# Shinokawa/Fast-SCNN-pytorch

Hardware: AMD Instinct MI355X
Metric: images/sec fwd+bwd @1024x2048 bs=8 per GPU; 1/2/4/8-GPU scaling (higher is better)
Workload: dtype bf16; 1 GPU; cfg3 train step: fwd + CE(ignore -1) + bwd + fused SGD (fused low-res upsample+CE head); model=FastSCNN (19 classes), global_batch=8, per_gpu_batch=8, parallelism=dp1

## Files before the change

fast-scnn-pytorch_amd/csrc/gemm_stream.hip:

```cpp
#include "bn_finish.hpp"

namespace fscnn {

constexpr int GS_MW = 32;
constexpr int GS_KMAX = 576;

template <typename T>
struct GsMma;
template <>
struct GsMma<float> {
  static __device__ __forceinline__ void run(const uint4& w, const uint4& x, f32x4& acc) {
    acc = __builtin_amdgcn_mfma_f32_16x16x4f32(__uint_as_float(w.x), __uint_as_float(x.x), acc, 0, 0, 0);
    acc = __builtin_amdgcn_mfma_f32_16x16x4f32(__uint_as_float(w.y), __uint_as_float(x.y), acc, 0, 0, 0);
    acc = __builtin_amdgcn_mfma_f32_16x16x4f32(__uint_as_float(w.z), __uint_as_float(x.z), acc, 0, 0, 0);
    acc = __builtin_amdgcn_mfma_f32_16x16x4f32(__uint_as_float(w.w), __uint_as_float(x.w), acc, 0, 0, 0);
  }
};
template <>
struct GsMma<bf16> {
  static __device__ __forceinline__ void run(const uint4& w, const uint4& x, f32x4& acc) {
    i16x8 wv, xv;
    __builtin_memcpy(&wv, &w, 16);
    __builtin_memcpy(&xv, &x, 16);
    acc = __builtin_amdgcn_mfma_f32_16x16x32_bf16(wv, xv, acc, 0, 0, 0);
  }
};
template <>
struct GsMma<f16> {
  static __device__ __forceinline__ void run(const uint4& w, const uint4& x, f32x4& acc) {
    h16x8 wv, xv;
    __builtin_memcpy(&wv, &w, 16);
    __builtin_memcpy(&xv, &x, 16);
    acc = __builtin_amdgcn_mfma_f32_16x16x32_f16(wv, xv, acc, 0, 0, 0);
  }
};

template <typename T>
__device__ __forceinline__ uint4 gs_tail(uint4 v, int valid) {
  constexpr int V = VecW<T>::V;
  uint32_t w[4] = {v.x, v.y, v.z, v.w};
#pragma unroll
  for (int j = 0; j < 4; ++j) {
    if (V == 4) {
      w[j] = j < valid ? w[j] : 0u;
    } else {
      const uint32_t lo = (2 * j < valid) ? 0x0000FFFFu : 0u;
      const uint32_t hi = (2 * j + 1 < valid) ? 0xFFFF0000u : 0u;
      w[j] &= lo | hi;
    }
  }
  return make_uint4(w[0], w[1], w[2], w[3]);
}

__device__ __forceinline__ float gs_rowsum(float v) {
  v += __shfl_xor(v, 1);
  v += __shfl_xor(v, 2);
  v += __shfl_xor(v, 4);
  v += __shfl_xor(v, 8);
  return v;
}

constexpr int GS_TEAM = 16;
constexpr int GS_CTR_TEAMS = 64;

template <bool FWD>
__device__ inline void gs_fold(const GemmArgs& a, int n0, int BN, int first, int count, int stride,
                               double (&sum)[3]) {
  __shared__ double s_f[3][256];
  const int tid = threadIdx.x;
  const int S = 256 / BN;
  const int col = tid % BN, sl = tid / BN;
  const int n = n0 + col;
  const int N = a.N;
  const float* base = FWD ? a.part : a.bpart;
  constexpr int R = FWD ? 3 : 2;
  constexpr int U = FWD ? 8 : 4;
  double t0 = 0.0, t1 = 0.0, t2 = 0.0;
  if (sl < S && n < N) {
    for (int i0 = sl; i0 < count; i0 += U * S) {
      float v[U][R];
#pragma unroll
      for (int u = 0; u < U; ++u) {
        const int i = i0 + u * S;
        const float* rec = base + (size_t)(first + (i < count ? i : i0) * stride) * R * N;
#pragma unroll
        for (int j = 0; j < R; ++j) v[u][j] = ld_wt(rec + (size_t)j * N + n);
      }
#pragma unroll
      for (int u = 0; u < U; ++u) {
        if (i0 + u * S >= count) break;
        if constexpr (FWD) {
          const double cn = v[u][2], m = v[u][0];
          t0 += cn;
          t1 += cn * m;
          t2 += (double)v[u][1] + cn * m * m;
        } else {
          t1 += v[u][0];
          t2 += v[u][1];
        }
      }
    }
  }
  s_f[0][tid] = t0;
  s_f[1][tid] = t1;
  s_f[2][tid] = t2;
  __syncthreads();
  sum[0] = sum[1] = sum[2] = 0.0;
  if (sl == 0) {
    for (int j = 0; j < S; ++j) {
      sum[0] += s_f[0][j * BN + col];
      sum[1] += s_f[1][j * BN + col];
      sum[2] += s_f[2][j * BN + col];
    }
  }
  __syncthreads();
}

template <bool FWD>
__device__ inline void gs_finish(const GemmArgs& a, int g, int bi, int n0, int BN, int bpg) {
  unsigned* ctr = a.tail.counters;
  const int team = bi / GS_TEAM, nteam = cdiv(bpg, GS_TEAM);
  const int tsize = min(GS_TEAM, bpg - team * GS_TEAM);
  const int tid = threadIdx.x, col = tid % BN, n = n0 + col;
  const bool owner = tid < BN && n < a.N;
  if (!arrive_last(ctr + GS_CTR_TEAMS + g * nteam + team, (unsigned)tsize)) return;
  BnFwdIn fin;
  BnBwdIn bin;
  if (owner) {
    if constexpr (FWD) fin = bn_fwd_load(a.tail.fwd, n);
    else bin = bn_bwd_load(a.tail.tab, n);
  }
  double s[3];
  gs_fold<FWD>(a, n0, BN, team * GS_TEAM, tsize, 1, s);
  if (owner) {
    const int N = a.N;
    if constexpr (FWD) {
      float* rec = a.part + (size_t)team * GS_TEAM * 3 * N;
      const double mean = s[0] > 0.0 ? s[1] / s[0] : 0.0;
      st_wt(rec + n, (float)mean);
      st_wt(rec + N + n, s[0] > 0.0 ? (float)fmax(s[2] - s[0] * mean * mean, 0.0) : 0.f);
      st_wt(rec + 2 * N + n, (float)s[0]);
    } else {
      float* rec = a.bpart + (size_t)team * GS_TEAM * 2 * N;
      st_wt(rec + n, (float)s[1]);
      st_wt(rec + N + n, (float)s[2]);
    }
  }
  reset_counter(ctr + GS_CTR_TEAMS + g * nteam + team);
  if (!arrive_last(ctr + g, (unsigned)nteam)) return;
  gs_fold<FWD>(a, n0, BN, 0, nteam, GS_TEAM, s);
  if (owner) {
    if constexpr (FWD) bn_fwd_finish(a.tail.fwd, n, s[0], s[1], s[2], fin);
    else bn_bwd_finish(n, a.N, s[1], s[2], a.tail.count, a.tail.dgamma, a.tail.dbeta,
                       a.tail.coef, a.tail.tab, bin);
  }
  reset_counter(ctr + g);
}

template <typename T, int NT, int KS, bool TAIL, bool AT, bool ST, bool BS>
__global__ __launch_bounds__(256, 2) void gemm_stream_kernel(GemmArgs a, int bpg) {
  constexpr int V = VecW<T>::V;
  constexpr int KV = 4 * KS;
  constexpr int KP = KV * V;
  constexpr int WST = KV + 1;
  constexpr int BN = 16 * NT;
  constexpr bool SUMS = ST || BS;
  extern __shared__ __attribute__((aligned(16))) uint4 s_w[];
  float* s_sc = reinterpret_cast<float*>(s_w + BN * WST);
  float* s_at = s_sc + 2 * BN;
  float* s_bc = s_at + (AT ? 2 * KP : 0);
  float* s_shf = s_bc + (BS ? 4 * BN : 0);

  const int tid = threadIdx.x, lane = tid & 63, wave = tid >> 6;
  const int li = lane & 15, lq = lane >> 4;
  const int g = blockIdx.x / bpg;
  const int bi = blockIdx.x - g * bpg;
  const int n0 = g * BN;
  const T* A = (const T*)a.A;
  const T* B = (const T*)a.B;
  stamp(a.stamps, 0);

  const int nchunks = cdiv(a.M, GS_MW);
  const int wstride = bpg * 4;
  int c = bi * 4 + wave;

  constexpr int NH =
      KS <= 4 ? 1 : (KS <= 8 ? 2 : (KS == 12 ? (BS ? 4 : 2) : (KS == 16 ? 4 : 6)));
  constexpr int KH = KS / NH;
  static_assert(KH * NH == KS && (NH == 1 || NH % 2 == 0), "k-steps split in an even part count");
  uint4 xa[2][KH], xn[2][KH];
  auto loadx = [&](int chunk, int h, uint4 (&r)[2][KH]) {
    const bool cok = chunk < nchunks;
#pragma unroll
    for (int mt = 0; mt < 2; ++mt) {
      const int m = chunk * GS_MW + mt * 16 + li;
      const bool mok = cok && m < a.M;
#pragma unroll
      for (int j = 0; j < KH; ++j) {
        const int k = (4 * (h * KH + j) + lq) * V;
        const bool ok = mok && k < a.K;
        r[mt][j] = *reinterpret_cast<const uint4*>(A + (ok ? (size_t)m * a.lda + k : 0));
      }
    }
  };

  if (c < nchunks) loadx(c, 0, xa);
  float t_sc = 1.f, t_sh = 0.f, t_bc[4] = {0.f, 0.f, 0.f, 1.f};
  if (tid < BN) {
    const int n = n0 + tid < a.N ? n0 + tid : 0;
    if (a.scale) t_sc = a.scale[n];
    if (a.shift) t_sh = a.shift[n];
    if constexpr (BS) {
      t_bc[0] = a.bmean[n];
      t_bc[1] = a.binvstd[n];
      if (a.bmode == 2) {
        t_bc[2] = a.bscale[n];
        t_bc[3] = a.bshift[n];
      }
    }
  }
  constexpr int ATI = AT ? (KP + 255) / 256 : 1;
  float t_at[ATI][2];
  if constexpr (AT) {
#pragma unroll
    for (int u = 0; u < ATI; ++u) {
      const int k = tid + u * 256;
      const bool ok = k < a.K;
      t_at[u][0] = ok ? a.a_scale[k] : 0.f;
      t_at[u][1] = ok ? a.a_shift[k] : 0.f;
    }
  }
  constexpr int WI = (BN * KV + 255) / 256;
  constexpr int WB = WI < 8 ? WI : 8;
#pragma unroll
  for (int u0 = 0; u0 < WI; u0 += WB) {
    uint4 t[WB];
#pragma unroll
    for (int u = 0; u < WB; ++u) {
      const int i = tid + (u0 + u) * 256;
      const int r = i / KV, v = i - r * KV;
      const int n = n0 + r, k = v * V;
      const bool ok = u0 + u < WI && i < BN * KV && n < a.N && k < a.K;
      t[u] = gs_tail<T>(*reinterpret_cast<const uint4*>(B + (ok ? (size_t)n * a.ldb + k : 0)),
                        ok ? a.K - k : 0);
    }
#pragma unroll
    for (int u = 0; u < WB; ++u) {
      const int i = tid + (u0 + u) * 256;
      const int r = i / KV, v = i - r * KV;
      if (u0 + u < WI && i < BN * KV) s_w[r * WST + v] = t[u];
    }
  }
  if (tid < BN) {
    s_sc[tid] = t_sc;
    s_sc[BN + tid] = t_sh;
    if constexpr (BS) {
#pragma unroll
      for (int j = 0; j < 4; ++j) s_bc[j * BN + tid] = t_bc[j];
    }
  }
  if constexpr (AT) {
#pragma unroll
    for (int u = 0; u < ATI; ++u) {
      const int k = tid + u * 256;
      if (k < KP) {
        s_at[k] = t_at[u][0];
        s_at[KP + k] = t_at[u][1];
      }
    }
  }
  __syncthreads();
  stamp(a.stamps, 1);

  float s1[SUMS ? NT : 1][4], s2[SUMS ? NT : 1][4];
  float cnt = 0.f;
  if constexpr (SUMS) {
#pragma unroll
    for (int nt = 0; nt < NT; ++nt)
#pragma unroll
      for (int r = 0; r < 4; ++r) { s1[nt][r] = 0.f; s2[nt][r] = 0.f; }
  }
  float* wshf = s_shf + wave * BN;
  if constexpr (ST) {
    for (int i = lane; i < BN; i += 64) wshf[i] = 0.f;
  }
  bool first = true;

  auto prep = [&](int chunk, int h, uint4 (&r)[2][KH]) {
#pragma unroll
    for (int mt = 0; mt < 2; ++mt) {
      const int m = chunk * GS_MW + mt * 16 + li;
      const bool mok = m < a.M;
#pragma unroll
      for (int j = 0; j < KH; ++j) {
        const int k = (4 * (h * KH + j) + lq) * V;
        uint4 v = r[mt][j];
        if constexpr (AT) v = bnrelu_vec<T>(v, s_at + k, s_at + KP + k);
        r[mt][j] = gs_tail<T>(v, mok ? a.K - k : 0);
      }
    }
  };

  T* Cp = (T*)a.C;
  const T* Rp = (const T*)a.R;
  constexpr bool DROP_OK = BS && KS == 1;
  const bool drop = DROP_OK && a.drop_hw != 0;
  const uint64_t dseed = drop ? (a.drop_seed_ptr ? *a.drop_seed_ptr : a.drop_seed) + a.drop_seed_add : 0;
  const float dscale = 1.f / (1.f - a.drop_p);
  for (; c < nchunks; c += wstride) {
    f32x4 acc[2][NT];
#pragma unroll
    for (int mt = 0; mt < 2; ++mt)
#pragma unroll
      for (int nt = 0; nt < NT; ++nt) acc[mt][nt] = f32x4{0.f, 0.f, 0.f, 0.f};
    int wb = li * WST + lq;
    asm volatile("" : "+v"(wb));
    const int wz = wb - li * WST - lq;
    const float* ssc = s_sc + wz;
    const float* sbc = s_bc + wz;
    auto mma = [&](int h, uint4 (&r)[2][KH]) {
#pragma unroll
      for (int j = 0; j < KH; ++j) {
#pragma unroll
        for (int nt = 0; nt < NT; ++nt) {
          const uint4 w = s_w[wb + nt * 16 * WST + 4 * (h * KH + j)];
#pragma unroll
          for (int mt = 0; mt < 2; ++mt) GsMma<T>::run(w, r[mt][j], acc[mt][nt]);
        }
      }
    };
    if constexpr (NH == 1) {
      loadx(c + wstride, 0, xn);
      prep(c, 0, xa);
      mma(0, xa);
    } else {
#pragma unroll
      for (int h = 0; h < NH; h += 2) {
        loadx(c, h + 1, xn);
        prep(c, h, xa);
        mma(h, xa);
        if (h + 2 < NH) loadx(c, h + 2, xa);
        else loadx(c + wstride, 0, xa);
        prep(c, h + 1, xn);
        mma(h + 1, xn);
      }
    }
    if constexpr (!TAIL) {
      if constexpr (ST) {
        if (first) {
          if (li == 0) {
#pragma unroll
            for (int nt = 0; nt < NT; ++nt) {
              const int nl = nt * 16 + 4 * lq;
#pragma unroll
              for (int r = 0; r < 4; ++r) wshf[nl + r] = acc[0][nt][r] * ssc[nl + r] + ssc[BN + nl + r];
            }
          }
          __builtin_amdgcn_wave_barrier();
          first = false;
        }
      }
#pragma unroll
      for (int mt = 0; mt < 2; ++mt) {
        const int m = c * GS_MW + mt * 16 + li;
        const bool mok = m < a.M;
        const size_t mr = mok ? (size_t)m : 0;
        float rv[NT][4];
        if (Rp) {
#pragma unroll
          for (int nt = 0; nt < NT; ++nt) ld4v(Rp + mr * a.ldr + n0 + nt * 16 + 4 * lq, rv[nt]);
        }
        float zv[BS ? NT : 1][4];
        if constexpr (BS) {
#pragma unroll
          for (int nt = 0; nt < NT; ++nt)
            ld4v((const T*)a.bz + mr * a.ldbz + n0 + nt * 16 + 4 * lq, zv[nt]);
        }
        if constexpr (SUMS) cnt += mok ? 1.f : 0.f;
#pragma unroll
        for (int nt = 0; nt < NT; ++nt) {
          const int nl = nt * 16 + 4 * lq;
          const float4 sc = *reinterpret_cast<const float4*>(ssc + nl);
          const float4 sh = *reinterpret_cast<const float4*>(ssc + BN + nl);
          const float scv[4] = {sc.x, sc.y, sc.z, sc.w}, shv[4] = {sh.x, sh.y, sh.z, sh.w};
          float shf[4] = {0.f, 0.f, 0.f, 0.f};
          if constexpr (ST) {
            const float4 t = *reinterpret_cast<const float4*>(wshf + wz + nl);
            shf[0] = t.x; shf[1] = t.y; shf[2] = t.z; shf[3] = t.w;
          }
          float o[4];
#pragma unroll
          for (int r = 0; r < 4; ++r) {
            float v = acc[mt][nt][r] * scv[r] + shv[r];
            if constexpr (ST) {
              const float d = mok ? round_as<T>(v) - shf[r] : 0.f;
              s1[nt][r] += d;
              s2[nt][r] += d * d;
            }
            if (Rp) v += rv[nt][r];
            o[r] = a.relu ? fmaxf(v, 0.f) : v;
          }
          if (DROP_OK && drop) {
            const unsigned HW = (unsigned)a.drop_hw;
            const unsigned pn = (unsigned)mr / HW, hw = (unsigned)mr - pn * HW;
#pragma unroll
            for (int r = 0; r < 4; ++r) {
              const uint64_t nchw = ((uint64_t)pn * a.N + (unsigned)(n0 + nl + r)) * HW + hw;
              o[r] = dropout_keep(dseed, nchw, a.drop_thr) ? round_as<T>(o[r]) * dscale : 0.f;
            }
          }
          if (mok) st4v(Cp + mr * a.ldc + n0 + nl, o);
          if constexpr (BS) {
            const float4 bm = *reinterpret_cast<const float4*>(sbc + nl);
            const float4 bv = *reinterpret_cast<const float4*>(sbc + BN + nl);
            const float4 bs = *reinterpret_cast<const float4*>(sbc + 2 * BN + nl);
            const float4 bh = *reinterpret_cast<const float4*>(sbc + 3 * BN + nl);
            const float bmv[4] = {bm.x, bm.y, bm.z, bm.w}, biv[4] = {bv.x, bv.y, bv.z, bv.w};
            const float bsv[4] = {bs.x, bs.y, bs.z, bs.w}, bhv[4] = {bh.x, bh.y, bh.z, bh.w};
#pragma unroll
            for (int r = 0; r < 4; ++r) {
              float gv = round_as<T>(o[r]);
              gv = (mok && fmaf(zv[nt][r], bsv[r], bhv[r]) > 0.f) ? gv : 0.f;
              s1[nt][r] += gv;
              s2[nt][r] += gv * (zv[nt][r] - bmv[r]) * biv[r];
            }
          }
        }
      }
    } else {
#pragma unroll
      for (int mt = 0; mt < 2; ++mt) {
        const int m = c * GS_MW + mt * 16 + li;
        if (m >= a.M) continue;
#pragma unroll
        for (int nt = 0; nt < NT; ++nt) {
          const int nl = nt * 16 + 4 * lq;
#pragma unroll
          for (int r = 0; r < 4; ++r) {
            const int n = n0 + nl + r;
            if (n >= a.N) continue;
            float v = acc[mt][nt][r] * ssc[nl + r] + ssc[BN + nl + r];
            if (Rp) v += ld1(Rp + (size_t)m * a.ldr + n);
            st1(Cp + (size_t)m * a.ldc + n, a.relu ? fmaxf(v, 0.f) : v);
          }
        }
      }
    }
    if constexpr (NH == 1) {
#pragma unroll
      for (int mt = 0; mt < 2; ++mt)
#pragma unroll
        for (int j = 0; j < KH; ++j) xa[mt][j] = xn[mt][j];
    }
  }

  stamp(a.stamps, 2);
  if constexpr (SUMS) {
    cnt = gs_rowsum(cnt);
    __syncthreads();
    float* red = reinterpret_cast<float*>(s_w);
#pragma unroll
    for (int nt = 0; nt < NT; ++nt)
#pragma unroll
      for (int r = 0; r < 4; ++r) {
        const float t1 = gs_rowsum(s1[nt][r]), t2 = gs_rowsum(s2[nt][r]);
        if (li == 0) {
          const int col = nt * 16 + 4 * lq + r;
          if constexpr (ST) {
            const float mean = cnt > 0.f ? wshf[col] + t1 / cnt : 0.f;
            const float m2 = cnt > 0.f ? fmaxf(t2 - t1 * (t1 / cnt), 0.f) : 0.f;
            red[(wave * 3 + 0) * BN + col] = cnt;
            red[(wave * 3 + 1) * BN + col] = mean;
            red[(wave * 3 + 2) * BN + col] = m2;
          } else {
            red[(wave * 3 + 0) * BN + col] = t1;
            red[(wave * 3 + 1) * BN + col] = t2;
          }
        }
      }
    __syncthreads();
    for (int col = tid; col < BN; col += 256) {
      const int n = n0 + col;
      if (n >= a.N) continue;
      if constexpr (ST) {
        float nn = 0.f, mean = 0.f, m2 = 0.f;
#pragma unroll
        for (int w = 0; w < 4; ++w) {
          const float nb = red[(w * 3 + 0) * BN + col];
          if (nb <= 0.f) continue;
          const float mb = red[(w * 3 + 1) * BN + col], qb = red[(w * 3 + 2) * BN + col];
          const float tot = nn + nb, d = mb - mean;
          mean += d * (nb / tot);
          m2 += qb + d * d * (nn * nb / tot);
          nn = tot;
        }
        float* rec = a.part + (size_t)bi * 3 * a.N;
        st_wt(rec + n, mean);
        st_wt(rec + a.N + n, m2);
        st_wt(rec + 2 * a.N + n, nn);
      } else {
        float t1 = 0.f, t2 = 0.f;
#pragma unroll
        for (int w = 0; w < 4; ++w) {
          t1 += red[(w * 3 + 0) * BN + col];
          t2 += red[(w * 3 + 1) * BN + col];
        }
        float* rec = a.bpart + (size_t)bi * 2 * a.N;
        st_wt(rec + n, t1);
        st_wt(rec + a.N + n, t2);
      }
    }
    stamp(a.stamps, 3);
    if (a.tail.counters) gs_finish<ST>(a, g, bi, n0, BN, bpg);
    stamp(a.stamps, 4);
  }
}

template <int NT, int KS, bool TAIL>
__global__ __launch_bounds__(256, 2) void gemm_stream_x3_kernel(GemmArgs a, int bpg) {
  constexpr int KV = 4 * KS;
  constexpr int WST = KV + 1;
  constexpr int BN = 16 * NT;
  extern __shared__ __attribute__((aligned(16))) uint4 s_w[];
  float* s_sc = reinterpret_cast<float*>(s_w + 3 * BN * WST);
  const int tid = threadIdx.x, lane = tid & 63, wave = tid >> 6;
  const int li = lane & 15, lq = lane >> 4;
  const int g = blockIdx.x / bpg;
  const int bi = blockIdx.x - g * bpg;
  const int n0 = g * BN;
  const float* A = (const float*)a.A;
  const float* B = (const float*)a.B;
  for (int i = tid; i < BN * KV; i += 256) {
    const int r = i / KV, v = i - r * KV;
    const int n = n0 + r, k = v * 8;
    const bool ok = n < a.N && k < a.K;
    const float* src = B + (ok ? (size_t)n * a.ldb + k : 0);
    const uint4 lo4 = gs_tail<float>(*reinterpret_cast<const uint4*>(src), ok ? a.K - k : 0);
    const uint4 hi4 = gs_tail<float>(*reinterpret_cast<const uint4*>(src + 4), ok ? a.K - k - 4 : 0);
    uint4 t[3];
    gs_split3(lo4, hi4, t);
#pragma unroll
    for (int j = 0; j < 3; ++j) s_w[(j * BN + r) * WST + v] = t[j];
  }
  for (int i = tid; i < BN; i += 256) {
    const int n = n0 + i < a.N ? n0 + i : 0;
    s_sc[i] = a.scale ? a.scale[n] : 1.f;
    s_sc[BN + i] = a.shift ? a.shift[n] : 0.f;
  }
  __syncthreads();

  const int nchunks = cdiv(a.M, GS_MW);
  const int wstride = bpg * 4;
  int c = bi * 4 + wave;
  uint4 xa[2][KS][2], xn[2][KS][2];
  auto loadx = [&](int chunk, uint4 (&r)[2][KS][2]) {
    const bool cok = chunk < nchunks;
#pragma unroll
    for (int mt = 0; mt < 2; ++mt) {
      const int m = chunk * GS_MW + mt * 16 + li;
      const bool mok = cok && m < a.M;
#pragma unroll
      for (int s = 0; s < KS; ++s)
#pragma unroll
        for (int h = 0; h < 2; ++h) {
          const int k = 32 * s + 8 * lq + 4 * h;
          const bool ok = mok && k < a.K;
          r[mt][s][h] = *reinterpret_cast<const uint4*>(A + (ok ? (size_t)m * a.lda + k : 0));
        }
    }
  };
  float* Cp = (float*)a.C;
  const float* Rp = (const float*)a.R;
  if (c < nchunks) loadx(c, xa);
  for (; c < nchunks; c += wstride) {
    loadx(c + wstride, xn);
    f32x4 acc[2][NT];
#pragma unroll
    for (int mt = 0; mt < 2; ++mt)
#pragma unroll
      for (int nt = 0; nt < NT; ++nt) acc[mt][nt] = f32x4{0.f, 0.f, 0.f, 0.f};
    int wb = li * WST + lq;
    asm volatile("" : "+v"(wb));
    const float* ssc = s_sc + (wb - li * WST - lq);
#pragma unroll
    for (int s = 0; s < KS; ++s) {
      uint4 xs[2][3];
#pragma unroll
      for (int mt = 0; mt < 2; ++mt) {
        const int m = c * GS_MW + mt * 16 + li;
        const bool mok = m < a.M;
        const int k = 32 * s + 8 * lq;
        gs_split3(gs_tail<float>(xa[mt][s][0], mok ? a.K - k : 0),
                  gs_tail<float>(xa[mt][s][1], mok ? a.K - k - 4 : 0), xs[mt]);
      }
#pragma unroll
      for (int nt = 0; nt < NT; ++nt) {
        uint4 w[3];
#pragma unroll
        for (int j = 0; j < 3; ++j) w[j] = s_w[(j * BN + nt * 16) * WST + wb + 4 * s];
#pragma unroll
        for (int mt = 0; mt < 2; ++mt) gs_mma_x3(w, xs[mt], acc[mt][nt]);
      }
    }
#pragma unroll
    for (int mt = 0; mt < 2; ++mt) {
      const int m = c * GS_MW + mt * 16 + li;
      const bool mok = m < a.M;
      const size_t mr = mok ? (size_t)m : 0;
      if constexpr (!TAIL) {
        float rv[NT][4];
        if (Rp) {
#pragma unroll
          for (int nt = 0; nt < NT; ++nt) ld4v(Rp + mr * a.ldr + n0 + nt * 16 + 4 * lq, rv[nt]);
        }
#pragma unroll
        for (int nt = 0; nt < NT; ++nt) {
          const int nl = nt * 16 + 4 * lq;
          float o[4];
#pragma unroll
          for (int r = 0; r < 4; ++r) {
            float v = acc[mt][nt][r] * ssc[nl + r] + ssc[BN + nl + r];
            if (Rp) v += rv[nt][r];
            o[r] = a.relu ? fmaxf(v, 0.f) : v;
          }
          if (mok) st4v(Cp + mr * a.ldc + n0 + nl, o);
        }
      } else {
        if (!mok) continue;
#pragma unroll
        for (int nt = 0; nt < NT; ++nt) {
          const int nl = nt * 16 + 4 * lq;
#pragma unroll
          for (int r = 0; r < 4; ++r) {
            const int n = n0 + nl + r;
            if (n >= a.N) continue;
            float v = acc[mt][nt][r] * ssc[nl + r] + ssc[BN + nl + r];
            if (Rp) v += ld1(Rp + (size_t)m * a.ldr + n);
            st1(Cp + (size_t)m * a.ldc + n, a.relu ? fmaxf(v, 0.f) : v);
          }
        }
      }
    }
#pragma unroll
    for (int mt = 0; mt < 2; ++mt)
#pragma unroll
      for (int s = 0; s < KS; ++s)
#pragma unroll
        for (int h = 0; h < 2; ++h) xa[mt][s][h] = xn[mt][s][h];
  }
}

static int gs_st_nt_cap() {
  static const int v = env_int("FSCNN_GS_ST_NT", 4);
  return v;
}

static int gs_pick_nt(const GemmArgs& a, int ks) {
  const int N = a.N;
  if (N <= 32) return 2;
  if (a.part && ks <= 8 && N > 64 && gs_st_nt_cap() > 0) {
    for (int nt = gs_st_nt_cap(); nt >= 2; --nt)
      if (N % (16 * nt) == 0) return nt;
  }
  if (ks > 8) return N % 64 == 0 ? 4 : (N % 48 == 0 ? 3 : 4);
  if (N <= 48) return 3;
  if (N <= 64 || a.bpart) return 4;
  if (a.part && ks > 2 && N % 64 == 0) return 4;
  if (N % 96 == 0) return 6;
  return a.part ? 4 : 8;
}

static bool gs_tail_needed(const GemmArgs& a, int nt) {
  return a.N % (16 * nt) != 0 || a.ldc % 4 != 0 || (a.R && a.ldr % 4 != 0);
}

static size_t gs_lds(const GemmArgs& a, int nt, int ks, int kc) {
  size_t b = (size_t)16 * nt * (4 * ks + 1) * 16 + (size_t)2 * 16 * nt * 4;
  if (a.a_scale) b += (size_t)2 * ks * kc * 4;
  if (a.bpart) b += (size_t)4 * 16 * nt * 4;
  if (a.part) b += (size_t)4 * 16 * nt * 4;
  return b;
}

static int gs_bpg(const GemmArgs& a, int dtype, int& nt, int& ks, size_t& lds);

bool gemm_stream_ok(const GemmArgs& a, int dtype) {
  const int KC = dtype == DT_F32 ? 16 : 32;
  const int ks = cdiv(a.K, KC);
  const bool sums = a.part || a.bpart;
  if (a.b_trans || (a.part && a.bpart)) return false;
  if (a.part && a.R) return false;
  if (a.a_scale && (!a.a_shift || !a.part || a.K > GS_KMAX)) return false;
  const bool deep = ks == 12 || ks == 16 || ks == 18;
  if (deep && dtype == DT_F32) return false;
  if (deep && a.M < 131072) return false;
  if (!(ks == 1 || ks == 2 || ks == 3 || ks == 4 || ks == 6 || ks == 8 || deep)) return false;
  const int nt = gs_pick_nt(a, ks);
  if (sums && ks > 4 && nt > 4) return false;
  if (sums && nt == 4 && ks > 12) return false;
  if (a.part && nt > 4 && ks > 2) return false;
  if (a.bpart && dtype == DT_F32 && nt == 4 && ks > 2) return false;
  if (gs_tail_needed(a, nt) && (nt != 2 || sums)) return false;
  if (a.bpart && (!a.bz || a.ldbz % 4 || (a.bmode != 0 && a.bmode != 2))) return false;
  if (a.drop_hw && (!a.bpart || ks != 1 || gs_tail_needed(a, nt) || a.M % a.drop_hw)) return false;
  if (gs_lds(a, nt, ks, KC) > (deep ? 80 * 1024 - 1024 : 72 * 1024)) return false;
  if (a.tail.counters) {
    int nt2, ks2;
    size_t lds2;
    const int bpg = gs_bpg(a, dtype, nt2, ks2, lds2);
    const int groups = cdiv(a.N, 16 * nt);
    if (groups > GS_CTR_TEAMS || GS_CTR_TEAMS + groups * cdiv(bpg, GS_TEAM) > BN_COUNTERS)
      return false;
  }
  return a.M >= 4096;
}

static int gs_fill_bpg(int slots, int groups) {
  const int b = slots / groups / 8 * 8;
  return b >= 8 ? b : (cdiv(slots, groups) + 7) / 8 * 8;
}

static int gs_bpg(const GemmArgs& a, int dtype, int& nt, int& ks, size_t& lds) {
  const int KC = dtype == DT_F32 ? 16 : 32;
  ks = cdiv(a.K, KC);
  nt = gs_pick_nt(a, ks);
  const int groups = cdiv(a.N, 16 * nt);
  lds = gs_lds(a, nt, ks, KC);
  const int nchunks = cdiv(a.M, GS_MW);
  constexpr int cap = 2;
  int per_cu = (int)((160 * 1024) / (lds + 1024));
  per_cu = per_cu < 1 ? 1 : (per_cu > cap ? cap : per_cu);
  int bpg = gs_fill_bpg(256 * per_cu, groups);
  const int need = cdiv(nchunks, 4);
  if (bpg > need) bpg = need;
  const int tmax = (BN_COUNTERS - GS_CTR_TEAMS) / groups * GS_TEAM;
  if (bpg > tmax) bpg = tmax;
  if (bpg < 1) bpg = 1;
  return bpg;
}

int gemm_stream_parts(const GemmArgs& a, int dtype) {
  int nt, ks;
  size_t lds;
  return gs_bpg(a, dtype, nt, ks, lds);
}

template <typename T, int NT, bool TAIL, bool AT, bool ST, bool BS>
static void gs_launch_ks(const GemmArgs& a, int ks, dim3 grid, size_t lds, int bpg,
                         hipStream_t st) {
  constexpr bool SUMS = ST || BS;
  constexpr bool WIDE = SUMS && NT > 4;
  constexpr bool DEEP = sizeof(T) == 2 && NT <= 4 && !TAIL;
  switch (ks) {
    case 1: prof_launch(gemm_stream_kernel<T, NT, 1, TAIL, AT, ST, BS>, grid, 256, lds, st, a, bpg); break;
    case 2: prof_launch(gemm_stream_kernel<T, NT, 2, TAIL, AT, ST, BS>, grid, 256, lds, st, a, bpg); break;
    case 3:
      if constexpr (!WIDE) prof_launch(gemm_stream_kernel<T, NT, 3, TAIL, AT, ST, BS>, grid, 256, lds, st, a, bpg);
      break;
    case 4:
      if constexpr (!WIDE) prof_launch(gemm_stream_kernel<T, NT, 4, TAIL, AT, ST, BS>, grid, 256, lds, st, a, bpg);
      break;
    case 6:
      if constexpr (!WIDE) prof_launch(gemm_stream_kernel<T, NT, 6, TAIL, AT, ST, BS>, grid, 256, lds, st, a, bpg);
      break;
    case 8:
      if constexpr (!WIDE) prof_launch(gemm_stream_kernel<T, NT, 8, TAIL, AT, ST, BS>, grid, 256, lds, st, a, bpg);
      break;
    default:
      if constexpr (DEEP) {
        if (ks == 12) prof_launch(gemm_stream_kernel<T, NT, 12, TAIL, AT, ST, BS>, grid, 256, lds, st, a, bpg);
        else if (ks == 16) prof_launch(gemm_stream_kernel<T, NT, 16, TAIL, AT, ST, BS>, grid, 256, lds, st, a, bpg);
        else prof_launch(gemm_stream_kernel<T, NT, 18, TAIL, AT, ST, BS>, grid, 256, lds, st, a, bpg);
      }
      break;
  }
}

template <typename T, bool AT, bool ST, bool BS>
static void gs_launch_nt(const GemmArgs& a, int nt, int ks, dim3 grid, size_t lds, int bpg,
                         hipStream_t st) {
  constexpr bool SUMS = ST || BS;
  switch (nt) {
    case 2:
      if (!SUMS && gs_tail_needed(a, nt)) gs_launch_ks<T, 2, true, AT, false, false>(a, ks, grid, lds, bpg, st);
      else gs_launch_ks<T, 2, false, AT, ST, BS>(a, ks, grid, lds, bpg, st);
      break;
    case 3: gs_launch_ks<T, 3, false, AT, ST, BS>(a, ks, grid, lds, bpg, st); break;
    case 4: gs_launch_ks<T, 4, false, AT, ST, BS>(a, ks, grid, lds, bpg, st); break;
    case 6:
      if constexpr (!BS) gs_launch_ks<T, 6, false, AT, ST, false>(a, ks, grid, lds, bpg, st);
      break;
    default:
      if constexpr (!SUMS) gs_launch_ks<T, 8, false, AT, false, false>(a, ks, grid, lds, bpg, st);
      break;
  }
}

template <typename T>
static void gs_launch(const GemmArgs& a, int dtype, hipStream_t st) {
  int nt, ks;
  size_t lds;
  const int bpg = gs_bpg(a, dtype, nt, ks, lds);
  const int groups = cdiv(a.N, 16 * nt);
  dim3 grid((unsigned)(groups * bpg));
  const bool at = a.a_scale != nullptr;
  if (a.bpart) gs_launch_nt<T, false, false, true>(a, nt, ks, grid, lds, bpg, st);
  else if (a.part && at) gs_launch_nt<T, true, true, false>(a, nt, ks, grid, lds, bpg, st);
  else if (a.part) gs_launch_nt<T, false, true, false>(a, nt, ks, grid, lds, bpg, st);
  else gs_launch_nt<T, false, false, false>(a, nt, ks, grid, lds, bpg, st);
}

static bool gs_x3_launch(const GemmArgs& a, hipStream_t st) {
  if (!f32_split_on() || a.part || a.bpart || a.a_scale || a.K > 128) return false;
  const int ks = cdiv(a.K, 32);
  auto lds_of = [&](int nt) { return (size_t)3 * 16 * nt * (4 * ks + 1) * 16 + (size_t)2 * 16 * nt * 4; };
  int nt = gs_pick_nt(a, ks);
  while (nt > 2 && lds_of(nt) > 72 * 1024) nt = nt == 8 ? 4 : (nt == 6 ? 3 : 2);
  if (lds_of(nt) > 72 * 1024) return false;
  const bool tail = gs_tail_needed(a, nt);
  if (tail && nt != 2) return false;
  const size_t lds = lds_of(nt);
  const int groups = cdiv(a.N, 16 * nt);
  int per_cu = (int)((160 * 1024) / (lds + 1024));
  per_cu = per_cu < 1 ? 1 : (per_cu > 2 ? 2 : per_cu);
  int bpg = gs_fill_bpg(256 * per_cu, groups);
  const int need = cdiv(cdiv(a.M, GS_MW), 4);
  if (bpg > need) bpg = need;
  if (bpg < 1) bpg = 1;
  const dim3 grid((unsigned)(groups * bpg));
#define X3(NT, KS, TL) prof_launch(gemm_stream_x3_kernel<NT, KS, TL>, grid, 256, lds, st, a, bpg)
#define X3K(NT, TL)                         \
  switch (ks) {                             \
    case 1: X3(NT, 1, TL); break;           \
    case 2: X3(NT, 2, TL); break;           \
    case 3: X3(NT, 3, TL); break;           \
    default: X3(NT, 4, TL); break;          \
  }
  switch (nt) {
    case 2: if (tail) { X3K(2, true) } else { X3K(2, false) } break;
    case 3: X3K(3, false) break;
    case 4: X3K(4, false) break;
    case 6: X3K(6, false) break;
    default: X3K(8, false) break;
  }
#undef X3K
#undef X3
  return true;
}

int gemm_stream(const GemmArgs& a, int dtype, hipStream_t st) {
  if (dtype == DT_F32) {
    if (!gs_x3_launch(a, st)) gs_launch<float>(a, dtype, st);
  } else if (dtype == DT_F16) {
    gs_launch<f16>(a, dtype, st);
  } else {
    gs_launch<bf16>(a, dtype, st);
  }
  return check_launch("gemm_stream");
}

}
```

Measured before the change: 1462 images/s.

## Add prefetching bf16 stream-GEMM variant for backward-stat kernels with 32-bit offsets

Adds a specialized gemm_stream_kernel_pf for bf16, non-tail, BS (backward stats) cases with KS<=12. It issues the epilogue operand loads (bz and residual rows) for the current chunk, and the next chunk's A loads, early so they overlap the MFMA work. Address arithmetic uses 32-bit offsets when the host check confirms the tensors fit under 4 GiB, and the epilogue uses vectorized row loads and stores. The added prefetch registers raise register pressure and may lower occupancy, and the code duplication adds maintenance cost.

```diff
diff --git a/fast-scnn-pytorch_amd/csrc/gemm_stream.hip b/fast-scnn-pytorch_amd/csrc/gemm_stream.hip
--- a/fast-scnn-pytorch_amd/csrc/gemm_stream.hip
+++ b/fast-scnn-pytorch_amd/csrc/gemm_stream.hip
@@ -2,6 +2,7 @@
 
 namespace fscnn {
 
+#define GS_INLINE __attribute__((always_inline))
 constexpr int GS_MW = 32;
 constexpr int GS_KMAX = 576;
 
@@ -50,6 +51,35 @@
     }
   }
   return make_uint4(w[0], w[1], w[2], w[3]);
+}
+
+template <typename P>
+__device__ __forceinline__ const P* gs_at(const P* base, uint32_t off) {
+  return reinterpret_cast<const P*>(reinterpret_cast<const char*>(base) +
+                                    (size_t)(off * (uint32_t)sizeof(P)));
+}
+template <typename P>
+__device__ __forceinline__ P* gs_at(P* base, uint32_t off) {
+  return reinterpret_cast<P*>(reinterpret_cast<char*>(base) + (size_t)(off * (uint32_t)sizeof(P)));
+}
+
+template <typename T> struct GsRow { using type = uint2; };
+template <> struct GsRow<float> { using type = uint4; };
+template <typename T>
+__device__ __forceinline__ typename GsRow<T>::type gs_row_load(const T* p) {
+  return *reinterpret_cast<const typename GsRow<T>::type*>(p);
+}
+__device__ __forceinline__ void gs_row_unpack(const float*, const uint4& t, float (&v)[4]) {
+  v[0] = __uint_as_float(t.x); v[1] = __uint_as_float(t.y);
+  v[2] = __uint_as_float(t.z); v[3] = __uint_as_float(t.w);
+}
+__device__ __forceinline__ void gs_row_unpack(const f16*, const uint2& t, float (&v)[4]) {
+  v[0] = h2f((uint16_t)(t.x & 0xFFFFu)); v[1] = h2f((uint16_t)(t.x >> 16));
+  v[2] = h2f((uint16_t)(t.y & 0xFFFFu)); v[3] = h2f((uint16_t)(t.y >> 16));
+}
+__device__ __forceinline__ void gs_row_unpack(const bf16*, const uint2& t, float (&v)[4]) {
+  v[0] = __uint_as_float(t.x << 16); v[1] = __uint_as_float(t.x & 0xFFFF0000u);
+  v[2] = __uint_as_float(t.y << 16); v[3] = __uint_as_float(t.y & 0xFFFF0000u);
 }
 
 __device__ __forceinline__ float gs_rowsum(float v) {
@@ -453,6 +483,380 @@
         for (int j = 0; j < KH; ++j) xa[mt][j] = xn[mt][j];
     }
   }
+
+  stamp(a.stamps, 2);
+  if constexpr (SUMS) {
+    cnt = gs_rowsum(cnt);
+    __syncthreads();
+    float* red = reinterpret_cast<float*>(s_w);
+#pragma unroll
+    for (int nt = 0; nt < NT; ++nt)
+#pragma unroll
+      for (int r = 0; r < 4; ++r) {
+        const float t1 = gs_rowsum(s1[nt][r]), t2 = gs_rowsum(s2[nt][r]);
+        if (li == 0) {
+          const int col = nt * 16 + 4 * lq + r;
+          if constexpr (ST) {
+            const float mean = cnt > 0.f ? wshf[col] + t1 / cnt : 0.f;
+            const float m2 = cnt > 0.f ? fmaxf(t2 - t1 * (t1 / cnt), 0.f) : 0.f;
+            red[(wave * 3 + 0) * BN + col] = cnt;
+            red[(wave * 3 + 1) * BN + col] = mean;
+            red[(wave * 3 + 2) * BN + col] = m2;
+          } else {
+            red[(wave * 3 + 0) * BN + col] = t1;
+            red[(wave * 3 + 1) * BN + col] = t2;
+          }
+        }
+      }
+    __syncthreads();
+    for (int col = tid; col < BN; col += 256) {
+      const int n = n0 + col;
+      if (n >= a.N) continue;
+      if constexpr (ST) {
+        float nn = 0.f, mean = 0.f, m2 = 0.f;
+#pragma unroll
+        for (int w = 0; w < 4; ++w) {
+          const float nb = red[(w * 3 + 0) * BN + col];
+          if (nb <= 0.f) continue;
+          const float mb = red[(w * 3 + 1) * BN + col], qb = red[(w * 3 + 2) * BN + col];
+          const float tot = nn + nb, d = mb - mean;
+          mean += d * (nb / tot);
+          m2 += qb + d * d * (nn * nb / tot);
+          nn = tot;
+        }
+        float* rec = a.part + (size_t)bi * 3 * a.N;
+        st_wt(rec + n, mean);
+        st_wt(rec + a.N + n, m2);
+        st_wt(rec + 2 * a.N + n, nn);
+      } else {
+        float t1 = 0.f, t2 = 0.f;
+#pragma unroll
+        for (int w = 0; w < 4; ++w) {
+          t1 += red[(w * 3 + 0) * BN + col];
+          t2 += red[(w * 3 + 1) * BN + col];
+        }
+        float* rec = a.bpart + (size_t)bi * 2 * a.N;
+        st_wt(rec + n, t1);
+        st_wt(rec + a.N + n, t2);
+      }
+    }
+    stamp(a.stamps, 3);
+    if (a.tail.counters) gs_finish<ST>(a, g, bi, n0, BN, bpg);
+    stamp(a.stamps, 4);
+  }
+}
+
+template <typename T, int NT, int KS, bool TAIL, bool BS>
+struct GsPf {
+  static constexpr bool value = BS && !TAIL && std::is_same<T, bf16>::value && KS <= 12;
+};
+
+template <typename T, int NT, int KS, bool TAIL, bool AT, bool ST, bool BS>
+__global__ __launch_bounds__(256, 2) void gemm_stream_kernel_pf(GemmArgs a, int bpg) {
+  constexpr int V = VecW<T>::V;
+  constexpr int KV = 4 * KS;
+  constexpr int KP = KV * V;
+  constexpr int WST = KV + 1;
+  constexpr int BN = 16 * NT;
+  constexpr bool SUMS = ST || BS;
+  extern __shared__ __attribute__((aligned(16))) uint4 s_w[];
+  float* s_sc = reinterpret_cast<float*>(s_w + BN * WST);
+  float* s_at = s_sc + 2 * BN;
+  float* s_bc = s_at + (AT ? 2 * KP : 0);
+  float* s_shf = s_bc + (BS ? 4 * BN : 0);
+
+  const int tid = threadIdx.x, lane = tid & 63, wave = tid >> 6;
+  const int li = lane & 15, lq = lane >> 4;
+  const int g = blockIdx.x / bpg;
+  const int bi = blockIdx.x - g * bpg;
+  const int n0 = g * BN;
+  const T* A = (const T*)a.A;
+  const T* B = (const T*)a.B;
+  stamp(a.stamps, 0);
+
+  const int nchunks = cdiv(a.M, GS_MW);
+  const int wstride = bpg * 4;
+  int c = bi * 4 + wave;
+
+  constexpr int NH =
+      KS <= 4 ? 1 : (KS <= 8 ? 2 : (KS == 12 ? (BS ? 4 : 2) : (KS == 16 ? 4 : 6)));
+  constexpr int KH = KS / NH;
+  static_assert(KH * NH == KS && (NH == 1 || NH % 2 == 0), "k-steps split in an even part count");
+  uint4 xa[2][KH], xn[2][KH];
+  auto loadx = [&](int chunk, int h, uint4 (&r)[2][KH]) GS_INLINE {
+    const bool cok = chunk < nchunks;
+#pragma unroll
+    for (int mt = 0; mt < 2; ++mt) {
+      const int m = chunk * GS_MW + mt * 16 + li;
+      const uint32_t row = (cok && m < a.M) ? (uint32_t)m * a.lda : 0u;
+#pragma unroll
+      for (int j = 0; j < KH; ++j) {
+        const int k = (4 * (h * KH + j) + lq) * V;
+        r[mt][j] = *reinterpret_cast<const uint4*>(gs_at(A, row + (k < a.K ? k : 0)));
+      }
+    }
+  };
+  static_assert(GsPf<T, NT, KS, TAIL, BS>::value, "a GsPf form");
+  using Row = typename GsRow<T>::type;
+  const T* Rp = (const T*)a.R;
+  const T* Zp = (const T*)a.bz;
+  Row zq[2][NT], rq[2][NT];
+  auto loade = [&](int chunk, Row (&z)[2][NT], Row (&r)[2][NT]) GS_INLINE {
+#pragma unroll
+    for (int mt = 0; mt < 2; ++mt) {
+      const int m = chunk * GS_MW + mt * 16 + li;
+      const uint32_t mr = (chunk < nchunks && m < a.M) ? (uint32_t)m : 0u;
+      const uint32_t cz = mr * a.ldbz + n0 + 4 * lq, cr = mr * a.ldr + n0 + 4 * lq;
+#pragma unroll
+      for (int nt = 0; nt < NT; ++nt) z[mt][nt] = gs_row_load<T>(gs_at(Zp, cz) + nt * 16);
+      if (Rp) {
+#pragma unroll
+        for (int nt = 0; nt < NT; ++nt) r[mt][nt] = gs_row_load<T>(gs_at(Rp, cr) + nt * 16);
+      }
+    }
+  };
+
+  if (c < nchunks) loadx(c, 0, xa);
+  float t_sc = 1.f, t_sh = 0.f, t_bc[4] = {0.f, 0.f, 0.f, 1.f};
+  if (tid < BN) {
+    const int n = n0 + tid < a.N ? n0 + tid : 0;
+    if (a.scale) t_sc = a.scale[n];
+    if (a.shift) t_sh = a.shift[n];
+    if constexpr (BS) {
+      t_bc[0] = a.bmean[n];
+      t_bc[1] = a.binvstd[n];
+      if (a.bmode == 2) {
+        t_bc[2] = a.bscale[n];
+        t_bc[3] = a.bshift[n];
+      }
+    }
+  }
+  constexpr int ATI = AT ? (KP + 255) / 256 : 1;
+  float t_at[ATI][2];
+  if constexpr (AT) {
+#pragma unroll
+    for (int u = 0; u < ATI; ++u) {
+      const int k = tid + u * 256;
+      const bool ok = k < a.K;
+      t_at[u][0] = ok ? a.a_scale[k] : 0.f;
+      t_at[u][1] = ok ? a.a_shift[k] : 0.f;
+    }
+  }
+  constexpr int WI = (BN * KV + 255) / 256;
+  constexpr int WB = WI < 8 ? WI : 8;
+#pragma unroll
+  for (int u0 = 0; u0 < WI; u0 += WB) {
+    uint4 t[WB];
+#pragma unroll
+    for (int u = 0; u < WB; ++u) {
+      const int i = tid + (u0 + u) * 256;
+      const int r = i / KV, v = i - r * KV;
+      const int n = n0 + r, k = v * V;
+      const bool ok = u0 + u < WI && i < BN * KV && n < a.N && k < a.K;
+      t[u] = gs_tail<T>(*reinterpret_cast<const uint4*>(B + (ok ? (size_t)n * a.ldb + k : 0)),
+                        ok ? a.K - k : 0);
+    }
+#pragma unroll
+    for (int u = 0; u < WB; ++u) {
+      const int i = tid + (u0 + u) * 256;
+      const int r = i / KV, v = i - r * KV;
+      if (u0 + u < WI && i < BN * KV) s_w[r * WST + v] = t[u];
+    }
+  }
+  if (tid < BN) {
+    s_sc[tid] = t_sc;
+    s_sc[BN + tid] = t_sh;
+    if constexpr (BS) {
+#pragma unroll
+      for (int j = 0; j < 4; ++j) s_bc[j * BN + tid] = t_bc[j];
+    }
+  }
+  if constexpr (AT) {
+#pragma unroll
+    for (int u = 0; u < ATI; ++u) {
+      const int k = tid + u * 256;
+      if (k < KP) {
+        s_at[k] = t_at[u][0];
+        s_at[KP + k] = t_at[u][1];
+      }
+    }
+  }
+  __syncthreads();
+  stamp(a.stamps, 1);
+
+  float s1[SUMS ? NT : 1][4], s2[SUMS ? NT : 1][4];
+  float cnt = 0.f;
+  if constexpr (SUMS) {
+#pragma unroll
+    for (int nt = 0; nt < NT; ++nt)
+#pragma unroll
+      for (int r = 0; r < 4; ++r) { s1[nt][r] = 0.f; s2[nt][r] = 0.f; }
+  }
+  float* wshf = s_shf + wave * BN;
+  if constexpr (ST) {
+    for (int i = lane; i < BN; i += 64) wshf[i] = 0.f;
+  }
+  bool first = true;
+
+  auto prep = [&](int chunk, int h, uint4 (&r)[2][KH], bool full) GS_INLINE {
+#pragma unroll
+    for (int mt = 0; mt < 2; ++mt) {
+      const int m = chunk * GS_MW + mt * 16 + li;
+      const bool mok = full || m < a.M;
+#pragma unroll
+      for (int j = 0; j < KH; ++j) {
+        const int k = (4 * (h * KH + j) + lq) * V;
+        uint4 v = r[mt][j];
+        if constexpr (AT) v = bnrelu_vec<T>(v, s_at + k, s_at + KP + k);
+        r[mt][j] = gs_tail<T>(v, mok ? a.K - k : 0);
+      }
+    }
+  };
+
+  T* Cp = (T*)a.C;
+  constexpr bool DROP_OK = BS && KS == 1;
+  const bool drop = DROP_OK && a.drop_hw != 0;
+  const uint64_t dseed = drop ? (a.drop_seed_ptr ? *a.drop_seed_ptr : a.drop_seed) + a.drop_seed_add : 0;
+  const float dscale = 1.f / (1.f - a.drop_p);
+  auto chunk = [&](auto full_c) GS_INLINE {
+    constexpr bool FULL = decltype(full_c)::value;
+    f32x4 acc[2][NT];
+#pragma unroll
+    for (int mt = 0; mt < 2; ++mt)
+#pragma unroll
+      for (int nt = 0; nt < NT; ++nt) acc[mt][nt] = f32x4{0.f, 0.f, 0.f, 0.f};
+    int wb = li * WST + lq;
+    asm volatile("" : "+v"(wb));
+    const int wz = wb - li * WST - lq;
+    const float* ssc = s_sc + wz;
+    const float* sbc = s_bc + wz;
+    auto mma = [&](int h, uint4 (&r)[2][KH]) GS_INLINE {
+#pragma unroll
+      for (int j = 0; j < KH; ++j) {
+#pragma unroll
+        for (int nt = 0; nt < NT; ++nt) {
+          const uint4 w = s_w[wb + nt * 16 * WST + 4 * (h * KH + j)];
+#pragma unroll
+          for (int mt = 0; mt < 2; ++mt) GsMma<T>::run(w, r[mt][j], acc[mt][nt]);
+        }
+      }
+    };
+    if constexpr (NH == 1) {
+      loade(c, zq, rq);
+      loadx(c + wstride, 0, xn);
+      prep(c, 0, xa, FULL);
+      mma(0, xa);
+    } else {
+#pragma unroll
+      for (int h = 0; h < NH; h += 2) {
+        loadx(c, h + 1, xn);
+        prep(c, h, xa, FULL);
+        mma(h, xa);
+        if (h + 2 < NH) {
+          loadx(c, h + 2, xa);
+        } else {
+          loade(c, zq, rq);
+          loadx(c + wstride, 0, xa);
+        }
+        prep(c, h + 1, xn, FULL);
+        mma(h + 1, xn);
+      }
+    }
+    if constexpr (!TAIL) {
+      if constexpr (ST) {
+        if (first) {
+          if (li == 0) {
+#pragma unroll
+            for (int nt = 0; nt < NT; ++nt) {
+              const int nl = nt * 16 + 4 * lq;
+#pragma unroll
+              for (int r = 0; r < 4; ++r) wshf[nl + r] = acc[0][nt][r] * ssc[nl + r] + ssc[BN + nl + r];
+            }
+          }
+          __builtin_amdgcn_wave_barrier();
+          first = false;
+        }
+      }
+      auto tile = [&](int mt, int nt, bool mok, uint32_t mr, uint32_t cc, f32x4 rv, f32x4 zv) GS_INLINE {
+        const int nl = nt * 16 + 4 * lq;
+        const float4 sc = *reinterpret_cast<const float4*>(ssc + nl);
+        const float4 sh = *reinterpret_cast<const float4*>(ssc + BN + nl);
+        const float scv[4] = {sc.x, sc.y, sc.z, sc.w}, shv[4] = {sh.x, sh.y, sh.z, sh.w};
+        float shf[4] = {0.f, 0.f, 0.f, 0.f};
+        if constexpr (ST) {
+          const float4 t = *reinterpret_cast<const float4*>(wshf + wz + nl);
+          shf[0] = t.x; shf[1] = t.y; shf[2] = t.z; shf[3] = t.w;
+        }
+        float o[4];
+#pragma unroll
+        for (int r = 0; r < 4; ++r) {
+          float v = acc[mt][nt][r] * scv[r] + shv[r];
+          if constexpr (ST) {
+            const float d = mok ? round_as<T>(v) - shf[r] : 0.f;
+            s1[nt][r] += d;
+            s2[nt][r] += d * d;
+          }
+          if (Rp) v += rv[r];
+          o[r] = a.relu ? fmaxf(v, 0.f) : v;
+        }
+        if (DROP_OK && drop) {
+          const unsigned HW = (unsigned)a.drop_hw;
+          const unsigned pn = mr / HW, hw = mr - pn * HW;
+#pragma unroll
+          for (int r = 0; r < 4; ++r) {
+            const uint64_t nchw = ((uint64_t)pn * a.N + (unsigned)(n0 + nl + r)) * HW + hw;
+            o[r] = dropout_keep(dseed, nchw, a.drop_thr) ? round_as<T>(o[r]) * dscale : 0.f;
+          }
+        }
+        if (mok) st4v(gs_at(Cp, cc) + nt * 16, o);
+        if constexpr (BS) {
+          const float4 bm = *reinterpret_cast<const float4*>(sbc + nl);
+          const float4 bv = *reinterpret_cast<const float4*>(sbc + BN + nl);
+          const float4 bs = *reinterpret_cast<const float4*>(sbc + 2 * BN + nl);
+          const float4 bh = *reinterpret_cast<const float4*>(sbc + 3 * BN + nl);
+          const float bmv[4] = {bm.x, bm.y, bm.z, bm.w}, biv[4] = {bv.x, bv.y, bv.z, bv.w};
+          const float bsv[4] = {bs.x, bs.y, bs.z, bs.w}, bhv[4] = {bh.x, bh.y, bh.z, bh.w};
+#pragma unroll
+          for (int r = 0; r < 4; ++r) {
+            float gv = round_as<T>(o[r]);
+            gv = (mok && fmaf(zv[r], bsv[r], bhv[r]) > 0.f) ? gv : 0.f;
+            s1[nt][r] += gv;
+            s2[nt][r] += gv * (zv[r] - bmv[r]) * biv[r];
+          }
+        }
+      };
+      bool mok[2];
+      uint32_t mr[2], cc[2];
+#pragma unroll
+      for (int mt = 0; mt < 2; ++mt) {
+        const int m = c * GS_MW + mt * 16 + li;
+        mok[mt] = FULL || m < a.M;
+        mr[mt] = mok[mt] ? (uint32_t)m : 0u;
+        cc[mt] = mr[mt] * a.ldc + n0 + 4 * lq;
+        cnt += mok[mt] ? 1.f : 0.f;
+      }
+#pragma unroll
+      for (int nt = 0; nt < NT; ++nt) {
+#pragma unroll
+        for (int mt = 0; mt < 2; ++mt) {
+          float rv[4] = {0.f, 0.f, 0.f, 0.f}, zv[4];
+          if (Rp) gs_row_unpack(Rp, rq[mt][nt], rv);
+          gs_row_unpack(Zp, zq[mt][nt], zv);
+          tile(mt, nt, mok[mt], mr[mt], cc[mt], f32x4{rv[0], rv[1], rv[2], rv[3]},
+               f32x4{zv[0], zv[1], zv[2], zv[3]});
+        }
+      }
+    }
+    if constexpr (NH == 1) {
+#pragma unroll
+      for (int mt = 0; mt < 2; ++mt)
+#pragma unroll
+        for (int j = 0; j < KH; ++j) xa[mt][j] = xn[mt][j];
+    }
+  };
+  const int nfull = a.M / GS_MW;
+  for (; c < nfull; c += wstride) chunk(std::true_type{});
+  if (c < nchunks) chunk(std::false_type{});
 
   stamp(a.stamps, 2);
   if constexpr (SUMS) {
@@ -745,6 +1149,23 @@
   return gs_bpg(a, dtype, nt, ks, lds);
 }
 
+static bool gs_pf_ok(const GemmArgs& a, size_t esz) {
+  const size_t lim = (size_t)1 << 32;
+  return (size_t)a.M * a.lda * esz < lim && (size_t)a.M * a.ldc * esz < lim &&
+         (!a.R || (size_t)a.M * a.ldr * esz < lim) && (size_t)a.M * a.ldbz * esz < lim;
+}
+
+template <typename T, int NT, int KS, bool TAIL, bool AT, bool ST, bool BS>
+static void gs_launch_form(const GemmArgs& a, dim3 grid, size_t lds, int bpg, hipStream_t st) {
+  if constexpr (GsPf<T, NT, KS, TAIL, BS>::value) {
+    if (gs_pf_ok(a, sizeof(T))) {
+      prof_launch(gemm_stream_kernel_pf<T, NT, KS, TAIL, AT, ST, BS>, grid, 256, lds, st, a, bpg);
+      return;
+    }
+  }
+  prof_launch(gemm_stream_kernel<T, NT, KS, TAIL, AT, ST, BS>, grid, 256, lds, st, a, bpg);
+}
+
 template <typename T, int NT, bool TAIL, bool AT, bool ST, bool BS>
 static void gs_launch_ks(const GemmArgs& a, int ks, dim3 grid, size_t lds, int bpg,
                          hipStream_t st) {
@@ -752,25 +1173,25 @@
   constexpr bool WIDE = SUMS && NT > 4;
   constexpr bool DEEP = sizeof(T) == 2 && NT <= 4 && !TAIL;
   switch (ks) {
-    case 1: prof_launch(gemm_stream_kernel<T, NT, 1, TAIL, AT, ST, BS>, grid, 256, lds, st, a, bpg); break;
-    case 2: prof_launch(gemm_stream_kernel<T, NT, 2, TAIL, AT, ST, BS>, grid, 256, lds, st, a, bpg); break;
+    case 1: gs_launch_form<T, NT, 1, TAIL, AT, ST, BS>(a, grid, lds, bpg, st); break;
+    case 2: gs_launch_form<T, NT, 2, TAIL, AT, ST, BS>(a, grid, lds, bpg, st); break;
     case 3:
-      if constexpr (!WIDE) prof_launch(gemm_stream_kernel<T, NT, 3, TAIL, AT, ST, BS>, grid, 256, lds, st, a, bpg);
+      if constexpr (!WIDE) gs_launch_form<T, NT, 3, TAIL, AT, ST, BS>(a, grid, lds, bpg, st);
       break;
     case 4:
-      if constexpr (!WIDE) prof_launch(gemm_stream_kernel<T, NT, 4, TAIL, AT, ST, BS>, grid, 256, lds, st, a, bpg);
+      if constexpr (!WIDE) gs_launch_form<T, NT, 4, TAIL, AT, ST, BS>(a, grid, lds, bpg, st);
       break;
     case 6:
-      if constexpr (!WIDE) prof_launch(gemm_stream_kernel<T, NT, 6, TAIL, AT, ST, BS>, grid, 256, lds, st, a, bpg);
+      if constexpr (!WIDE) gs_launch_form<T, NT, 6, TAIL, AT, ST, BS>(a, grid, lds, bpg, st);
       break;
     case 8:
-      if constexpr (!WIDE) prof_launch(gemm_stream_kernel<T, NT, 8, TAIL, AT, ST, BS>, grid, 256, lds, st, a, bpg);
+      if constexpr (!WIDE) gs_launch_form<T, NT, 8, TAIL, AT, ST, BS>(a, grid, lds, bpg, st);
       break;
     default:
       if constexpr (DEEP) {
-        if (ks == 12) prof_launch(gemm_stream_kernel<T, NT, 12, TAIL, AT, ST, BS>, grid, 256, lds, st, a, bpg);
-        else if (ks == 16) prof_launch(gemm_stream_kernel<T, NT, 16, TAIL, AT, ST, BS>, grid, 256, lds, st, a, bpg);
-        else prof_launch(gemm_stream_kernel<T, NT, 18, TAIL, AT, ST, BS>, grid, 256, lds, st, a, bpg);
+        if (ks == 12) gs_launch_form<T, NT, 12, TAIL, AT, ST, BS>(a, grid, lds, bpg, st);
+        else if (ks == 16) gs_launch_form<T, NT, 16, TAIL, AT, ST, BS>(a, grid, lds, bpg, st);
+        else gs_launch_form<T, NT, 18, TAIL, AT, ST, BS>(a, grid, lds, bpg, st);
       }
       break;
   }
```

Result: no change. 1474 images/s, median of 6 (+0.8%).
